# wx-ys/pynbody-extras

Measured on AMD Instinct MI355X. Metric: particle-pairs/sec (direct-sum gravity, force+potential), higher is better.
Workload: dtype f64; 1 GPU; 1000000-particle Plummer sphere, direct-sum force+potential (Newtonian), 1000000 targets/GPU x 1000000 sources; n_particles=1000000, seed=1002, parallelism=targets sharded x1, device=gfx950 device (gfx950:sramecc+:xnack-, 256 CUs)

## Files before the change

pynbody-extras_amd/csrc/direct.hip:

```cpp
#include <cstdlib>
#include <cstring>

#include "pbx_common.h"

namespace pbx {

static constexpr double kR2Tiny = 2.2250738585072014e-308;
static constexpr int kBlock = 256;

__device__ __forceinline__ double rsqrt_nr(double x) {
  double y = __builtin_amdgcn_rsq(x);
  double e = __builtin_fma(-x * y, y, 1.0);
  return __builtin_fma(0.5 * y, e, y);
}

__device__ __forceinline__ double w2_inner(double u) {
  double u2 = u * u;
  if (u < 0.5) {
    double u4 = u2 * u2;
    double u5 = u4 * u;
    return (16.0 / 3.0) * u2 - (48.0 / 5.0) * u4 + (32.0 / 5.0) * u5 - 14.0 / 5.0;
  }
  double inv_u = 1.0 / u;
  double u3 = u2 * u;
  double u4 = u2 * u2;
  double u5 = u4 * u;
  return (1.0 / 15.0) * inv_u + (32.0 / 3.0) * u2 - 16.0 * u3 + (48.0 / 5.0) * u4 -
         (32.0 / 15.0) * u5 - 16.0 / 5.0;
}

__device__ __forceinline__ double w2p_inner(double u) {
  double u2 = u * u;
  double u3 = u2 * u;
  double u4 = u2 * u2;
  if (u < 0.5) return (32.0 / 3.0) * u - (192.0 / 5.0) * u3 + 32.0 * u4;
  return -(1.0 / 15.0) * (1.0 / u2) + (64.0 / 3.0) * u - 48.0 * u2 + (192.0 / 5.0) * u3 -
         (32.0 / 3.0) * u4;
}

template <int KERN, int WANT>
__device__ __forceinline__ void pair(double dx, double dy, double dz, double m, double h,
                                     double &ph, double &ax, double &ay, double &az) {
  double s2 = __builtin_fma(dx, dx, __builtin_fma(dy, dy, __builtin_fma(dz, dz, kR2Tiny)));
  const double s = (KERN == 0) ? __builtin_fma(h, h, s2) : s2;
  const double y0 = __builtin_amdgcn_rsq(s);
  const double w = y0 * __builtin_fma(-s, y0 * y0, 3.0);
  double mw = m * w;
  double g8 = mw * (w * w);
  if (KERN == 1) {
    double r = s2 * (0.5 * w);
    if (!(h <= 0.0) && !(r >= h)) {
      double hinv = 1.0 / h;
      double u = r * hinv;
      mw = -2.0 * m * (w2_inner(u) * hinv);
      g8 = 8.0 * m * (w2p_inner(u) * (hinv * hinv) / r);
    }
  }
  if (WANT & PBX_WANT_POT) ph += mw;
  if (WANT & PBX_WANT_ACC) {
    ax = __builtin_fma(g8, dx, ax);
    ay = __builtin_fma(g8, dy, ay);
    az = __builtin_fma(g8, dz, az);
  }
}

template <int KERN, int WANT, bool CHECK, int T>
__device__ __forceinline__ void sweep(const double4 *__restrict__ src,
                                      const double *__restrict__ src_h, bool has_h,
                                      int64_t j0, int64_t j1, const double (&xi)[T],
                                      const double (&yi)[T], const double (&zi)[T],
                                      const double (&hi)[T], const int64_t (&me)[T],
                                      double (&ph)[T], double (&ax)[T], double (&ay)[T],
                                      double (&az)[T]) {
#pragma unroll 4
  for (int64_t j = j0; j < j1; ++j) {
    const double4 s = src[j];
    double hj = 0.0;
    if (KERN >= 0) hj = has_h ? src_h[j] : 0.0;
#pragma unroll
    for (int k = 0; k < T; ++k) {
      double dx = s.x - xi[k];
      double dy = s.y - yi[k];
      double dz = s.z - zi[k];
      double m = s.w;
      double h = 0.0;
      if (KERN >= 0) h = __builtin_fmax(hi[k], hj);
      if (CHECK) {
        bool self = (j == me[k]);
        m = self ? 0.0 : m;
        dx = self ? 1.0 : dx;
        if (KERN >= 0) h = self ? 0.0 : h;
      }
      pair<KERN, WANT>(dx, dy, dz, m, h, ph[k], ax[k], ay[k], az[k]);
    }
  }
}

template <int KERN, int WANT, bool SELF, int T>
__global__ void __launch_bounds__(kBlock)
    direct_kernel(const double4 *__restrict__ src, const double *__restrict__ src_h,
                  int has_h, int64_t n_src, int64_t chunk, const double *__restrict__ tgt,
                  const double *__restrict__ tgt_h, int64_t n_tgt, int64_t self_offset,
                  double *__restrict__ pot_out, double *__restrict__ acc_out,
                  int64_t out_split_stride) {
  const int64_t tbase = (int64_t)blockIdx.x * (kBlock * T);
  const int64_t js = (int64_t)blockIdx.y * chunk;
  const int64_t je = (js + chunk < n_src) ? js + chunk : n_src;

  double xi[T], yi[T], zi[T], hi[T], ph[T], ax[T], ay[T], az[T];
  int64_t me[T];
#pragma unroll
  for (int k = 0; k < T; ++k) {
    int64_t t = tbase + k * kBlock + threadIdx.x;
    int64_t tc = t < n_tgt ? t : n_tgt - 1;
    xi[k] = tgt[3 * tc + 0];
    yi[k] = tgt[3 * tc + 1];
    zi[k] = tgt[3 * tc + 2];
    hi[k] = (SELF && KERN >= 0 && has_h) ? tgt_h[tc] : 0.0;
    me[k] = SELF ? self_offset + t : -1;
    ph[k] = ax[k] = ay[k] = az[k] = 0.0;
  }

  const bool hh = has_h != 0;
  if (SELF) {
    int64_t d0 = self_offset + tbase;
    int64_t d1 = d0 + kBlock * T;
    d0 = d0 < js ? js : (d0 > je ? je : d0);
    d1 = d1 < js ? js : (d1 > je ? je : d1);
    sweep<KERN, WANT, false, T>(src, src_h, hh, js, d0, xi, yi, zi, hi, me, ph, ax, ay, az);
    sweep<KERN, WANT, true, T>(src, src_h, hh, d0, d1, xi, yi, zi, hi, me, ph, ax, ay, az);
    sweep<KERN, WANT, false, T>(src, src_h, hh, d1, je, xi, yi, zi, hi, me, ph, ax, ay, az);
  } else {
    sweep<KERN, WANT, false, T>(src, src_h, hh, js, je, xi, yi, zi, hi, me, ph, ax, ay, az);
  }

  const int64_t soff = (int64_t)blockIdx.y * out_split_stride;
#pragma unroll
  for (int k = 0; k < T; ++k) {
    int64_t t = tbase + k * kBlock + threadIdx.x;
    if (t < n_tgt) {
      if (WANT & PBX_WANT_POT) pot_out[soff + t] = -0.5 * ph[k];
      if (WANT & PBX_WANT_ACC) {
        double *a = acc_out + 3 * (soff + t);
        a[0] = 0.125 * ax[k];
        a[1] = 0.125 * ay[k];
        a[2] = 0.125 * az[k];
      }
    }
  }
}

template <int WANT>
__global__ void __launch_bounds__(kBlock)
    reduce_splits(const double *__restrict__ pot_part, const double *__restrict__ acc_part,
                  int nsplit, int64_t n_tgt, double *__restrict__ pot,
                  double *__restrict__ acc) {
  int64_t t = (int64_t)blockIdx.x * kBlock + threadIdx.x;
  if (t >= n_tgt) return;
  if (WANT & PBX_WANT_POT) {
    double s = 0.0;
    for (int k = 0; k < nsplit; ++k) s += pot_part[(int64_t)k * n_tgt + t];
    pot[t] = s;
  }
  if (WANT & PBX_WANT_ACC) {
    double sx = 0.0, sy = 0.0, sz = 0.0;
    for (int k = 0; k < nsplit; ++k) {
      const double *a = acc_part + 3 * ((int64_t)k * n_tgt + t);
      sx += a[0];
      sy += a[1];
      sz += a[2];
    }
    acc[3 * t + 0] = sx;
    acc[3 * t + 1] = sy;
    acc[3 * t + 2] = sz;
  }
}

__global__ void __launch_bounds__(kBlock)
    pack_sources_kernel(const double *__restrict__ pos, const double *__restrict__ mass,
                        int64_t n, double4 *__restrict__ rec) {
  int64_t i = (int64_t)blockIdx.x * kBlock + threadIdx.x;
  if (i >= n) return;
  rec[i] = make_double4(pos[3 * i + 0], pos[3 * i + 1], pos[3 * i + 2],
                        mass ? mass[i] : 1.0);
}

constexpr int kTargetsPerLane = 4;

template <int KERN, int WANT, bool SELF>
static void launch_variant(hipStream_t st, dim3 grid, const double4 *src, const double *src_h,
                           int has_h, int64_t n_src, int64_t chunk, const double *tgt,
                           const double *tgt_h, int64_t n_tgt, int64_t self_offset,
                           double *pot, double *acc, int64_t stride) {
  hipLaunchKernelGGL((direct_kernel<KERN, WANT, SELF, kTargetsPerLane>), grid, dim3(kBlock), 0,
                     st, src, src_h, has_h, n_src, chunk, tgt, tgt_h, n_tgt, self_offset, pot, acc,
                     stride);
}

template <int KERN, int WANT>
static void launch_self(bool self, hipStream_t st, dim3 grid, const double4 *src,
                        const double *src_h, int has_h, int64_t n_src, int64_t chunk,
                        const double *tgt, const double *tgt_h, int64_t n_tgt,
                        int64_t self_offset, double *pot, double *acc, int64_t stride) {
  if (self)
    launch_variant<KERN, WANT, true>(st, grid, src, src_h, has_h, n_src, chunk, tgt, tgt_h,
                                     n_tgt, self_offset, pot, acc, stride);
  else
    launch_variant<KERN, WANT, false>(st, grid, src, src_h, has_h, n_src, chunk, tgt, tgt_h,
                                      n_tgt, self_offset, pot, acc, stride);
}

template <int KERN>
static void launch_want(int want, bool self, hipStream_t st, dim3 grid, const double4 *src,
                        const double *src_h, int has_h, int64_t n_src, int64_t chunk,
                        const double *tgt, const double *tgt_h, int64_t n_tgt,
                        int64_t self_offset, double *pot, double *acc, int64_t stride) {
  switch (want) {
    case 1:
      launch_self<KERN, 1>(self, st, grid, src, src_h, has_h, n_src, chunk, tgt, tgt_h, n_tgt,
                           self_offset, pot, acc, stride);
      break;
    case 2:
      launch_self<KERN, 2>(self, st, grid, src, src_h, has_h, n_src, chunk, tgt, tgt_h, n_tgt,
                           self_offset, pot, acc, stride);
      break;
    default:
      launch_self<KERN, 3>(self, st, grid, src, src_h, has_h, n_src, chunk, tgt, tgt_h, n_tgt,
                           self_offset, pot, acc, stride);
      break;
  }
}

int64_t sym_padded(int64_t n);
int64_t sym_unit_count(int64_t n);
void sym_accumulate(Device &d, double4 *rec, int64_t n, int64_t u0, int64_t u1, int want,
                    double *acc4, DevBuf &unit_buf);
void sym_finish(Device &d, const double *acc4, int64_t lo, int64_t hi, int want, double *pot,
                double *acc);

static constexpr int64_t kSymMinN = 8192;

void direct_device(Device &d, const double *src, const double *src_h, int64_t n_src,
                   const double *tgt, const double *tgt_h, int64_t n_tgt, int64_t self_offset,
                   int kernel, int want, double *pot, double *acc) {
  if (n_tgt <= 0) return;
  hipStream_t st = d.stream;
  if (kernel == PBX_KERNEL_NONE && self_offset == 0 && n_tgt == n_src && n_src >= kSymMinN) {
    const int64_t npad = sym_padded(n_src);
    double4 *rec = (double4 *)d.slot(kSlotSymRec).ensure(sizeof(double4) * npad);
    double *acc4 = (double *)d.slot(kSlotSymAcc).ensure(sizeof(double) * 4 * npad);
    PBX_HIP(hipMemcpyAsync(rec, src, sizeof(double4) * n_src, hipMemcpyDeviceToDevice, st));
    PBX_HIP(hipMemsetAsync(acc4, 0, sizeof(double) * 4 * npad, st));
    sym_accumulate(d, rec, n_src, 0, sym_unit_count(n_src), want, acc4, d.slot(kSlotSymUnits));
    sym_finish(d, acc4, 0, n_src, want, pot, acc);
    return;
  }
  if (n_src <= 0) {
    if (want & PBX_WANT_POT) PBX_HIP(hipMemsetAsync(pot, 0, sizeof(double) * n_tgt, st));
    if (want & PBX_WANT_ACC) PBX_HIP(hipMemsetAsync(acc, 0, sizeof(double) * 3 * n_tgt, st));
    return;
  }
  const int64_t per_block = (int64_t)kBlock * kTargetsPerLane;
  const int64_t bx = (n_tgt + per_block - 1) / per_block;
  int64_t nsplit = (2048 + bx - 1) / bx;
  int64_t max_split = (n_src + 4095) / 4096;
  if (nsplit > max_split) nsplit = max_split;
  if (nsplit > 64) nsplit = 64;
  if (nsplit < 1) nsplit = 1;
  const int64_t chunk = (n_src + nsplit - 1) / nsplit;
  nsplit = (n_src + chunk - 1) / chunk;
  if (bx > 0x7fffffff) fail(PBX_ERR_VALUE, "too many targets (%lld)", (long long)n_tgt);
  dim3 grid((unsigned)bx, (unsigned)nsplit);
  const bool self = self_offset >= 0;
  const int has_h = src_h != nullptr;

  double *pot_k = pot, *acc_k = acc;
  int64_t stride = 0;
  if (nsplit > 1) {
    size_t per = 0;
    if (want & PBX_WANT_POT) per += 1;
    if (want & PBX_WANT_ACC) per += 3;
    double *part = (double *)d.slot(kSlotPart).ensure(sizeof(double) * per * nsplit * n_tgt);
    pot_k = (want & PBX_WANT_POT) ? part : nullptr;
    acc_k = (want & PBX_WANT_ACC) ? part + ((want & PBX_WANT_POT) ? nsplit * n_tgt : 0)
                                  : nullptr;
    stride = n_tgt;
  }
  const double4 *src4 = (const double4 *)src;
  switch (kernel) {
    case PBX_KERNEL_NONE:
      launch_want<-1>(want, self, st, grid, src4, src_h, has_h, n_src, chunk, tgt, tgt_h,
                      n_tgt, self_offset, pot_k, acc_k, stride);
      break;
    case PBX_KERNEL_PLUMMER:
      launch_want<0>(want, self, st, grid, src4, src_h, has_h, n_src, chunk, tgt, tgt_h,
                     n_tgt, self_offset, pot_k, acc_k, stride);
      break;
    case PBX_KERNEL_SPLINE:
      launch_want<1>(want, self, st, grid, src4, src_h, has_h, n_src, chunk, tgt, tgt_h,
                     n_tgt, self_offset, pot_k, acc_k, stride);
      break;
    default:
      fail(PBX_ERR_VALUE, "kernel must be 0 (Plummer) or 1 (CubicSplineW2)");
  }
  PBX_HIP(hipGetLastError());
  if (nsplit > 1) {
    dim3 rg(ceil_div(n_tgt, kBlock));
    switch (want) {
      case 1:
        hipLaunchKernelGGL(reduce_splits<1>, rg, dim3(kBlock), 0, st, pot_k, acc_k,
                           (int)nsplit, n_tgt, pot, acc);
        break;
      case 2:
        hipLaunchKernelGGL(reduce_splits<2>, rg, dim3(kBlock), 0, st, pot_k, acc_k,
                           (int)nsplit, n_tgt, pot, acc);
        break;
      default:
        hipLaunchKernelGGL(reduce_splits<3>, rg, dim3(kBlock), 0, st, pot_k, acc_k,
                           (int)nsplit, n_tgt, pot, acc);
        break;
    }
    PBX_HIP(hipGetLastError());
  }
}

void pack_sources_device(Device &d, const double *pos, const double *mass, int64_t n,
                         double *rec) {
  if (n <= 0) return;
  hipLaunchKernelGGL(pack_sources_kernel, dim3(ceil_div(n, kBlock)), dim3(kBlock), 0, d.stream,
                     pos, mass, n, (double4 *)rec);
  PBX_HIP(hipGetLastError());
}

static void check_kernel(int kernel, const double *soft) {
  if (kernel != PBX_KERNEL_NONE && kernel != PBX_KERNEL_PLUMMER && kernel != PBX_KERNEL_SPLINE)
    fail(PBX_ERR_VALUE, "kernel must be 0 (Plummer) or 1 (CubicSplineW2)");
  if (kernel == PBX_KERNEL_NONE && soft != nullptr)
    fail(PBX_ERR_VALUE,
         "softenings require an explicit kernel; pass kernel=0/1 (or omit softenings)");
}

static void direct_host(const double *h_pos, int64_t n, const double *h_tgt, int64_t m,
                        const double *h_mass, const double *h_soft, int kernel, int want,
                        double *h_out) {
  if (n < 0 || m < 0) fail(PBX_ERR_VALUE, "negative particle count");
  check_kernel(kernel, h_soft);
  const bool self = (h_tgt == nullptr);
  const int64_t n_tgt = self ? n : m;
  if (n_tgt == 0) return;
  Device &d = current_device();
  std::lock_guard<std::mutex> lk(d.mu);
  hipStream_t st = d.stream;
  size_t out_elems = (want == PBX_WANT_POT ? 1 : 3) * (size_t)n_tgt;
  if (n == 0) {
    std::memset(h_out, 0, sizeof(double) * out_elems);
    return;
  }
  ScopedTimer total("pbx.direct.total");
  double *d_pos = (double *)d.slot(kSlotPos).ensure(sizeof(double) * 3 * n);
  double *d_mass = h_mass ? (double *)d.slot(kSlotMass).ensure(sizeof(double) * n) : nullptr;
  double *d_src = (double *)d.slot(kSlotSrc).ensure(sizeof(double) * 4 * n);
  const bool use_h = h_soft != nullptr && kernel != PBX_KERNEL_NONE;
  double *d_src_h = use_h ? (double *)d.slot(kSlotSrcH).ensure(sizeof(double) * n) : nullptr;
  double *d_tgt = self ? d_pos : (double *)d.slot(kSlotTgt).ensure(sizeof(double) * 3 * m);
  double *d_out = (double *)d.slot(want == PBX_WANT_POT ? kSlotPot : kSlotAcc)
                      .ensure(sizeof(double) * out_elems);
  {
    ScopedTimer t("pbx.direct.h2d");
    PBX_HIP(hipMemcpyAsync(d_pos, h_pos, sizeof(double) * 3 * n, hipMemcpyHostToDevice, st));
    if (h_mass)
      PBX_HIP(hipMemcpyAsync(d_mass, h_mass, sizeof(double) * n, hipMemcpyHostToDevice, st));
    if (use_h)
      PBX_HIP(hipMemcpyAsync(d_src_h, h_soft, sizeof(double) * n, hipMemcpyHostToDevice, st));
    if (!self)
      PBX_HIP(hipMemcpyAsync(d_tgt, h_tgt, sizeof(double) * 3 * m, hipMemcpyHostToDevice, st));
    if (timing_enabled()) PBX_HIP(hipStreamSynchronize(st));
  }
  {
    ScopedTimer t("pbx.direct.compute");
    pack_sources_device(d, d_pos, d_mass, n, d_src);
    direct_device(d, d_src, d_src_h, n, d_tgt, self ? d_src_h : nullptr, n_tgt,
                  self ? 0 : -1, kernel, want, want == PBX_WANT_POT ? d_out : nullptr,
                  want == PBX_WANT_ACC ? d_out : nullptr);
    if (timing_enabled()) PBX_HIP(hipStreamSynchronize(st));
  }
  {
    ScopedTimer t("pbx.direct.d2h");
    PBX_HIP(hipMemcpyAsync(h_out, d_out, sizeof(double) * out_elems, hipMemcpyDeviceToHost, st));
    PBX_HIP(hipStreamSynchronize(st));
  }
}

}

using namespace pbx;

extern "C" {

int pbx_direct_accelerations(const double *h_pos, int64_t n, const double *h_masses,
                             const double *h_softenings, int kernel, double *h_acc) {
  return guard([&] {
    direct_host(h_pos, n, nullptr, 0, h_masses, h_softenings, kernel, PBX_WANT_ACC, h_acc);
  });
}

int pbx_direct_potentials(const double *h_pos, int64_t n, const double *h_masses,
                          const double *h_softenings, int kernel, double *h_pot) {
  return guard([&] {
    direct_host(h_pos, n, nullptr, 0, h_masses, h_softenings, kernel, PBX_WANT_POT, h_pot);
  });
}

int pbx_direct_accelerations_at_points(const double *h_pos, int64_t n, const double *h_targets,
                                       int64_t m, const double *h_masses,
                                       const double *h_softenings, int kernel, double *h_acc) {
  return guard([&] {
    if (m > 0 && !h_targets) fail(PBX_ERR_VALUE, "targets must be (N,3) float64 array");
    direct_host(h_pos, n, h_targets ? h_targets : h_pos, m, h_masses, h_softenings, kernel,
                PBX_WANT_ACC, h_acc);
  });
}

int pbx_direct_potentials_at_points(const double *h_pos, int64_t n, const double *h_targets,
                                    int64_t m, const double *h_masses,
                                    const double *h_softenings, int kernel, double *h_pot) {
  return guard([&] {
    if (m > 0 && !h_targets) fail(PBX_ERR_VALUE, "targets must be (N,3) float64 array");
    direct_host(h_pos, n, h_targets ? h_targets : h_pos, m, h_masses, h_softenings, kernel,
                PBX_WANT_POT, h_pot);
  });
}

int pbx_pack_sources(const double *d_pos, const double *d_mass, int64_t n, double *d_records) {
  return guard([&] {
    if (n < 0) fail(PBX_ERR_VALUE, "negative particle count");
    Device &d = current_device();
    pack_sources_device(d, d_pos, d_mass, n, d_records);
  });
}

int pbx_direct_dev(const double *d_src, const double *d_src_h, int64_t n_src,
                   const double *d_tgt, const double *d_tgt_h, int64_t n_tgt,
                   int64_t self_offset, int kernel, int want, double *d_pot, double *d_acc) {
  return guard([&] {
    if (n_src < 0 || n_tgt < 0) fail(PBX_ERR_VALUE, "negative particle count");
    if (want < 1 || want > 3) fail(PBX_ERR_VALUE, "want must be 1 (pot), 2 (acc) or 3");
    if ((want & PBX_WANT_POT) && !d_pot && n_tgt) fail(PBX_ERR_VALUE, "d_pot is NULL");
    if ((want & PBX_WANT_ACC) && !d_acc && n_tgt) fail(PBX_ERR_VALUE, "d_acc is NULL");
    if (kernel != PBX_KERNEL_NONE && kernel != PBX_KERNEL_PLUMMER && kernel != PBX_KERNEL_SPLINE)
      fail(PBX_ERR_VALUE, "kernel must be 0 (Plummer) or 1 (CubicSplineW2)");
    if (self_offset >= 0 && self_offset + n_tgt > n_src)
      fail(PBX_ERR_VALUE, "self_offset + n_tgt exceeds n_src");
    if (self_offset >= 0 && kernel != PBX_KERNEL_NONE && d_src_h && !d_tgt_h)
      fail(PBX_ERR_VALUE, "all-particles softened form needs d_tgt_h");
    Device &d = current_device();
    std::lock_guard<std::mutex> lk(d.mu);
    direct_device(d, d_src, kernel == PBX_KERNEL_NONE ? nullptr : d_src_h, n_src, d_tgt,
                  d_tgt_h, n_tgt, self_offset, kernel, want, d_pot, d_acc);
  });
}

}
```

pynbody-extras_amd/csrc/direct_sym.hip:

```cpp
#include <algorithm>
#include <type_traits>
#include <vector>

#include "pbx_common.h"

namespace pbx {
namespace sym {

static constexpr double kR2Tiny = 2.2250738585072014e-308;
constexpr int kWaves = 4;
#ifndef PBX_SYM_KT
#define PBX_SYM_KT 12
#endif
#ifndef PBX_SYM_KS
#define PBX_SYM_KS 2
#endif
constexpr int kT = PBX_SYM_KT;
constexpr int kS = PBX_SYM_KS;
constexpr int kBlk = 64 * kT;
constexpr int kChunk = 64 * kS;
constexpr int kJPerI = kBlk / kChunk;
constexpr int kSuper = kWaves * kBlk;
static_assert(kJPerI * kChunk == kBlk, "an I-block is a whole number of J-chunks");

struct Unit {
  int32_t sb;
  int32_t j0;
  int32_t j1;
  int32_t pad;
};

__device__ __forceinline__ double rot(double v, int addr) {
  const uint64_t b = __builtin_bit_cast(uint64_t, v);
  const int lo = __builtin_amdgcn_ds_bpermute(addr, (int)(uint32_t)b);
  const int hi = __builtin_amdgcn_ds_bpermute(addr, (int)(uint32_t)(b >> 32));
  return __builtin_bit_cast(double, ((uint64_t)(uint32_t)hi << 32) | (uint64_t)(uint32_t)lo);
}

__device__ __forceinline__ double rot_dpp(double v) {
  const uint64_t b = __builtin_bit_cast(uint64_t, v);
  const int l0 = (int)(uint32_t)b, h0 = (int)(uint32_t)(b >> 32);
  const int lo = __builtin_amdgcn_update_dpp(l0, l0, 0x134, 0xF, 0xF, false);
  const int hi = __builtin_amdgcn_update_dpp(h0, h0, 0x134, 0xF, 0xF, false);
  return __builtin_bit_cast(double, ((uint64_t)(uint32_t)hi << 32) | (uint64_t)(uint32_t)lo);
}
#ifndef PBX_SYM_DPP_MASK
#define PBX_SYM_DPP_MASK 0xFF
#endif

template <int WANT, bool SYMM, bool RAW, bool UNI, int DOFF = 0>
__device__ __forceinline__ void chunk(const double4 *__restrict__ rec, int64_t jbase, int lane,
                                      const double (&tx)[kT], const double (&ty)[kT],
                                      const double (&tz)[kT], const double (&tm)[kT],
                                      double (&tp)[kT], double (&ta)[kT], double (&tb)[kT],
                                      double (&tc)[kT], double (&sp)[kS], double (&sa)[kS],
                                      double (&sb)[kS], double (&sc)[kS]) {
  double sx[kS], sy[kS], sz[kS], sm[kS];
#pragma unroll
  for (int k = 0; k < kS; ++k) {
    const double4 r = rec[jbase + k * 64 + lane];
    sx[k] = r.x;
    sy[k] = r.y;
    sz[k] = r.z;
    sm[k] = UNI ? 0.0 : r.w;
    sp[k] = sa[k] = sb[k] = sc[k] = 0.0;
  }
  const int addr = ((lane + 1) & 63) << 2;
  for (int r = 0; r < 64; ++r) {
#pragma unroll
    for (int ks = 0; ks < kS; ++ks) {
#pragma unroll
      for (int kt = 0; kt < kT; ++kt) {
        double dx = sx[ks] - tx[kt], dy = sy[ks] - ty[kt], dz = sz[ks] - tz[kt];
        double ms = sm[ks];
        bool self = false;
        if (!SYMM && kt == DOFF * kS + ks) {
          self = (r == 0);
          ms = self ? 0.0 : ms;
          dx = self ? 1.0 : dx;
        }
        const double s2 =
            __builtin_fma(dx, dx, __builtin_fma(dy, dy, __builtin_fma(dz, dz, kR2Tiny)));
        const double y0 = __builtin_amdgcn_rsq(s2);
        double w = RAW ? y0 : y0 * __builtin_fma(-s2, y0 * y0, 3.0);
        if (UNI && !SYMM && kt == DOFF * kS + ks) w = self ? 0.0 : w;
        const double q = w * (w * w);
        if (WANT & PBX_WANT_POT) tp[kt] = UNI ? tp[kt] + w : __builtin_fma(ms, w, tp[kt]);
        if (WANT & PBX_WANT_ACC) {
          const double g = UNI ? q : ms * q;
          ta[kt] = __builtin_fma(g, dx, ta[kt]);
          tb[kt] = __builtin_fma(g, dy, tb[kt]);
          tc[kt] = __builtin_fma(g, dz, tc[kt]);
        }
        if (SYMM) {
          if (WANT & PBX_WANT_POT) sp[ks] = UNI ? sp[ks] + w : __builtin_fma(tm[kt], w, sp[ks]);
          if (WANT & PBX_WANT_ACC) {
            const double g = UNI ? q : tm[kt] * q;
            sa[ks] = __builtin_fma(-g, dx, sa[ks]);
            sb[ks] = __builtin_fma(-g, dy, sb[ks]);
            sc[ks] = __builtin_fma(-g, dz, sc[ks]);
          }
        }
      }
      auto rt = [&](double x, int bit) {
        return ((PBX_SYM_DPP_MASK >> bit) & 1) ? rot_dpp(x) : rot(x, addr);
      };
      sx[ks] = rt(sx[ks], 0);
      sy[ks] = rt(sy[ks], 1);
      sz[ks] = rt(sz[ks], 2);
      if (!UNI) sm[ks] = rt(sm[ks], 3);
      if (SYMM) {
        if (WANT & PBX_WANT_POT) sp[ks] = rt(sp[ks], 4);
        if (WANT & PBX_WANT_ACC) {
          sa[ks] = rt(sa[ks], 5);
          sb[ks] = rt(sb[ks], 6);
          sc[ks] = rt(sc[ks], 7);
        }
      }
    }
  }
}

template <int WANT, bool RAW, bool UNI, int D>
__device__ __forceinline__ void own_chunk(int d, const double4 *__restrict__ rec, int64_t jbase,
                                          int lane, const double (&tx)[kT], const double (&ty)[kT],
                                          const double (&tz)[kT], const double (&tm)[kT],
                                          double (&tp)[kT], double (&ta)[kT], double (&tb)[kT],
                                          double (&tc)[kT], double (&sp)[kS], double (&sa)[kS],
                                          double (&sb)[kS], double (&sc)[kS]) {
  if (d == D)
    chunk<WANT, false, RAW, UNI, D>(rec, jbase, lane, tx, ty, tz, tm, tp, ta, tb, tc, sp, sa, sb, sc);
  else if constexpr (D + 1 < kJPerI)
    own_chunk<WANT, RAW, UNI, D + 1>(d, rec, jbase, lane, tx, ty, tz, tm, tp, ta, tb, tc, sp, sa, sb,
                                     sc);
}

template <int WANT, bool RAW, bool UNI>
__global__ void __launch_bounds__(kWaves * 64)
    sym_kernel(const double4 *__restrict__ rec, const Unit *__restrict__ units,
               double *__restrict__ acc4, double m) {
  __shared__ double jl[kWaves][4][kChunk];
  const Unit u = units[blockIdx.x];
  const int w = threadIdx.x >> 6, lane = threadIdx.x & 63;
  const int64_t iblk = (int64_t)u.sb * kWaves + w;
  double tx[kT], ty[kT], tz[kT], tm[kT], tp[kT], ta[kT], tb[kT], tc[kT];
#pragma unroll
  for (int k = 0; k < kT; ++k) {
    const double4 r = rec[iblk * kBlk + k * 64 + lane];
    tx[k] = r.x;
    ty[k] = r.y;
    tz[k] = r.z;
    tm[k] = UNI ? 0.0 : r.w;
    tp[k] = ta[k] = tb[k] = tc[k] = 0.0;
  }
  const int64_t jdiag = iblk * kJPerI;
  for (int32_t j = u.j0; j < u.j1; ++j) {
    double sp[kS], sa[kS], sb[kS], sc[kS];
#pragma unroll
    for (int k = 0; k < kS; ++k) sp[k] = sa[k] = sb[k] = sc[k] = 0.0;
    if (j >= jdiag + kJPerI)
      chunk<WANT, true, RAW, UNI>(rec, (int64_t)j * kChunk, lane, tx, ty, tz, tm, tp, ta, tb, tc, sp,
                                  sa, sb, sc);
    else if (j >= jdiag)
      own_chunk<WANT, RAW, UNI, 0>((int)(j - jdiag), rec, (int64_t)j * kChunk, lane, tx, ty, tz, tm,
                                   tp, ta, tb, tc, sp, sa, sb, sc);
#pragma unroll
    for (int k = 0; k < kS; ++k) {
      jl[w][0][k * 64 + lane] = sp[k];
      jl[w][1][k * 64 + lane] = sa[k];
      jl[w][2][k * 64 + lane] = sb[k];
      jl[w][3][k * 64 + lane] = sc[k];
    }
    __syncthreads();
    if ((int64_t)j >= ((int64_t)u.sb * kWaves + 1) * kJPerI) {
      double *dst = acc4 + (int64_t)j * kChunk * 4;
      static_assert(kWaves * 64 * kS == kChunk * 4, "kS (source, quantity) words per thread");
#pragma unroll
      for (int i = 0; i < kS; ++i) {
        const int idx = threadIdx.x + i * kWaves * 64;
        const int s = idx >> 2, q = idx & 3;
        double v = jl[0][q][s] + jl[1][q][s] + jl[2][q][s] + jl[3][q][s];
        if (UNI) v *= m;
        if (v != 0.0) atomicAdd(dst + idx, v);
      }
    }
    __syncthreads();
  }
#pragma unroll
  for (int k = 0; k < kT; ++k) {
    double *dst = acc4 + (iblk * kBlk + k * 64 + lane) * 4;
    if (WANT & PBX_WANT_POT) atomicAdd(dst + 0, UNI ? m * tp[k] : tp[k]);
    if (WANT & PBX_WANT_ACC) {
      atomicAdd(dst + 1, UNI ? m * ta[k] : ta[k]);
      atomicAdd(dst + 2, UNI ? m * tb[k] : tb[k]);
      atomicAdd(dst + 3, UNI ? m * tc[k] : tc[k]);
    }
  }
}

__global__ void pad_records(double4 *__restrict__ rec, int64_t n, int64_t npad) {
  int64_t i = n + (int64_t)blockIdx.x * 256 + threadIdx.x;
  if (i >= npad) return;
  const double far = 1e100 * (double)(i - n + 1);
  rec[i] = make_double4(far, -far, 2.0 * far, 0.0);
}

struct MassProbe {
  double m;
  uint32_t differs;
  uint32_t pad;
};
__global__ void mass_probe(const double4 *__restrict__ rec, int64_t n,
                           MassProbe *__restrict__ out) {
  const int64_t i = (int64_t)blockIdx.x * 256 + threadIdx.x;
  const double m0 = rec[0].w;
  if (i == 0) out->m = m0;
  if (i < n && __builtin_bit_cast(uint64_t, rec[i].w) != __builtin_bit_cast(uint64_t, m0))
    out->differs = 1u;
}

__global__ void finish_kernel(const double *__restrict__ acc4, int64_t lo, int64_t hi, int want,
                              int raw, double *__restrict__ pot, double *__restrict__ acc) {
  int64_t t = (int64_t)blockIdx.x * 256 + threadIdx.x;
  if (lo + t >= hi) return;
  const double *a = acc4 + (lo + t) * 4;
  const double kp = raw ? -1.0 : -0.5, ka = raw ? 1.0 : 0.125;
  if (want & PBX_WANT_POT) pot[t] = kp * a[0];
  if (want & PBX_WANT_ACC) {
    acc[3 * t + 0] = ka * a[1];
    acc[3 * t + 1] = ka * a[2];
    acc[3 * t + 2] = ka * a[3];
  }
}

}

int64_t sym_padded(int64_t n) {
  return (n + sym::kSuper - 1) / sym::kSuper * sym::kSuper;
}

#ifndef PBX_SYM_CHUNKS_PER_UNIT
#define PBX_SYM_CHUNKS_PER_UNIT 32
#endif
static std::vector<sym::Unit> sym_units(int64_t npad) {
  constexpr int kChunksPerUnit = PBX_SYM_CHUNKS_PER_UNIT;
  const int32_t nch = (int32_t)(npad / sym::kChunk);
  const int32_t nsb = (int32_t)(npad / sym::kSuper);
  std::vector<sym::Unit> u;
  for (int32_t sb = 0; sb < nsb; ++sb)
    for (int32_t j = sb * sym::kWaves * sym::kJPerI; j < nch; j += kChunksPerUnit)
      u.push_back({sb, j, std::min(nch, j + kChunksPerUnit), 0});
  return u;
}

int64_t sym_unit_count(int64_t n) { return (int64_t)sym_units(sym_padded(n)).size(); }

static sym::MassProbe sym_probe_mass(Device &d, const double4 *rec, int64_t n) {
  hipStream_t st = d.stream;
  sym::MassProbe *dp = (sym::MassProbe *)d.slot(kSlotSymProbe).ensure(sizeof(sym::MassProbe));
  sym::MassProbe h{};
  const bool timed = timing_enabled();
  hipEvent_t e0 = nullptr, e1 = nullptr;
  if (timed) {
    PBX_HIP(hipEventCreate(&e0));
    PBX_HIP(hipEventCreate(&e1));
    PBX_HIP(hipEventRecord(e0, st));
  }
  PBX_HIP(hipMemsetAsync(dp, 0, sizeof(sym::MassProbe), st));
  hipLaunchKernelGGL(sym::mass_probe, dim3(ceil_div(n, 256)), dim3(256), 0, st, rec, n, dp);
  PBX_HIP(hipGetLastError());
  PBX_HIP(hipMemcpyAsync(&h, dp, sizeof(sym::MassProbe), hipMemcpyDeviceToHost, st));
  if (timed) PBX_HIP(hipEventRecord(e1, st));
  PBX_HIP(hipStreamSynchronize(st));
  if (timed) {
    float ms = 0.f;
    PBX_HIP(hipEventElapsedTime(&ms, e0, e1));
    std::fprintf(stderr, "[pynbodyext-timing] direct_sym mass probe (n=%lld): %.4f ms\n",
                 (long long)n, (double)ms);
    (void)hipEventDestroy(e0);
    (void)hipEventDestroy(e1);
  }
  return h;
}


void sym_accumulate(Device &d, double4 *rec, int64_t n, int64_t u0, int64_t u1, int want,
                    double *acc4, DevBuf &unit_buf) {
  const int64_t npad = sym_padded(n);
  hipStream_t st = d.stream;
  if (npad > n)
    hipLaunchKernelGGL(sym::pad_records, dim3(ceil_div(npad - n, 256)), dim3(256), 0, st, rec, n,
                       npad);
  std::vector<sym::Unit> all = sym_units(npad);
  u0 = std::max<int64_t>(0, u0);
  u1 = std::min<int64_t>((int64_t)all.size(), u1);
  if (u1 <= u0) return;
  std::vector<sym::Unit> mine(all.begin() + u0, all.begin() + u1);
  std::stable_sort(mine.begin(), mine.end(), [](const sym::Unit &a, const sym::Unit &b) {
    return (a.j1 - a.j0) > (b.j1 - b.j0);
  });
  sym::Unit *du = (sym::Unit *)unit_buf.ensure(sizeof(sym::Unit) * mine.size());
  PBX_HIP(hipMemcpyAsync(du, mine.data(), sizeof(sym::Unit) * mine.size(), hipMemcpyHostToDevice,
                         st));
  const sym::MassProbe probe = sym_probe_mass(d, rec, n);
  const bool uni = probe.differs == 0;
  const double m = probe.m;
  const dim3 grid((unsigned)mine.size()), block(sym::kWaves * 64);
  auto launch = [&](auto raw, auto uniform) {
    constexpr bool R = decltype(raw)::value, U = decltype(uniform)::value;
    if (want == PBX_WANT_POT)
      hipLaunchKernelGGL((sym::sym_kernel<PBX_WANT_POT, R, U>), grid, block, 0, st, rec, du, acc4,
                         m);
    else if (want == PBX_WANT_ACC)
      hipLaunchKernelGGL((sym::sym_kernel<PBX_WANT_ACC, R, U>), grid, block, 0, st, rec, du, acc4,
                         m);
    else
      hipLaunchKernelGGL((sym::sym_kernel<PBX_WANT_POT | PBX_WANT_ACC, R, U>), grid, block, 0, st,
                         rec, du, acc4, m);
  };
  auto launch_raw = [&](auto raw) {
    if (uni)
      launch(raw, std::true_type{});
    else
      launch(raw, std::false_type{});
  };
  if (precise_mode())
    launch_raw(std::false_type{});
  else
    launch_raw(std::true_type{});
  ++(uni ? d.sym_uniform_launches : d.sym_general_launches);
  PBX_HIP(hipGetLastError());
  PBX_HIP(hipStreamSynchronize(st));
}

void sym_finish(Device &d, const double *acc4, int64_t lo, int64_t hi, int want, double *pot,
                double *acc) {
  if (hi <= lo) return;
  hipLaunchKernelGGL(sym::finish_kernel, dim3(ceil_div(hi - lo, 256)), dim3(256), 0, d.stream,
                     acc4, lo, hi, want, precise_mode() ? 0 : 1, pot, acc);
  PBX_HIP(hipGetLastError());
}

}

using namespace pbx;

extern "C" {

int pbx_direct_sym_plan(int64_t n, int64_t *npad, int64_t *n_units, int64_t *h_weights) {
  return guard([&] {
    if (n < 0) fail(PBX_ERR_VALUE, "negative particle count");
    const int64_t np = sym_padded(n);
    std::vector<sym::Unit> u = sym_units(np);
    if (npad) *npad = np;
    if (n_units) *n_units = (int64_t)u.size();
    if (h_weights)
      for (size_t i = 0; i < u.size(); ++i) h_weights[i] = u[i].j1 - u[i].j0;
  });
}

int pbx_direct_sym_accumulate(const double *d_src, int64_t n, int64_t u0, int64_t u1, int want,
                              double *d_acc4) {
  return guard([&] {
    if (n < 0) fail(PBX_ERR_VALUE, "negative particle count");
    if (want < 1 || want > 3) fail(PBX_ERR_VALUE, "want must be 1 (pot), 2 (acc) or 3");
    if (n == 0) return;
    Device &d = current_device();
    std::lock_guard<std::mutex> lk(d.mu);
    const int64_t npad = sym_padded(n);
    double4 *rec = (double4 *)d.slot(kSlotSymRec).ensure(sizeof(double4) * npad);
    PBX_HIP(hipMemcpyAsync(rec, d_src, sizeof(double4) * n, hipMemcpyDeviceToDevice, d.stream));
    sym_accumulate(d, rec, n, u0, u1, want, d_acc4, d.slot(kSlotSymUnits));
  });
}

int pbx_direct_sym_path_stats(int64_t *uniform_launches, int64_t *general_launches) {
  return guard([&] {
    Device &d = current_device();
    std::lock_guard<std::mutex> lk(d.mu);
    if (uniform_launches) *uniform_launches = d.sym_uniform_launches;
    if (general_launches) *general_launches = d.sym_general_launches;
  });
}

int pbx_direct_sym_finish(const double *d_acc4, int64_t lo, int64_t hi, int want, double *d_pot,
                          double *d_acc) {
  return guard([&] {
    if (lo < 0 || hi < lo) fail(PBX_ERR_VALUE, "bad particle range");
    Device &d = current_device();
    std::lock_guard<std::mutex> lk(d.mu);
    sym_finish(d, d_acc4, lo, hi, want, d_pot, d_acc);
    PBX_HIP(hipStreamSynchronize(d.stream));
  });
}

}
```

pynbody-extras_amd/csrc/pbx_common.h:

```cpp
#pragma once

#include <hip/hip_runtime.h>

#include <chrono>
#include <condition_variable>
#include <cstdarg>
#include <cstdint>
#include <cstdio>
#include <mutex>
#include <string>
#include <thread>
#include <vector>

#include "../../include/pbx.h"

namespace pbx {

void set_error(const char *fmt, ...);

struct Error {
  int code;
  std::string msg;
};

[[noreturn]] void fail(int code, const char *fmt, ...);

#define PBX_HIP(call)                                                        \
  do {                                                                       \
    hipError_t _e = (call);                                                  \
    if (_e != hipSuccess)                                                    \
      ::pbx::fail(PBX_ERR_RUNTIME, "%s failed: %s (%s:%d)", #call,           \
                  hipGetErrorString(_e), __FILE__, __LINE__);                \
  } while (0)

template <class F> int guard(F &&f) {
  try {
    f();
    return PBX_OK;
  } catch (const Error &e) {
    set_error("%s", e.msg.c_str());
    return e.code;
  } catch (const std::bad_alloc &) {
    set_error("host allocation failed");
    return PBX_ERR_RUNTIME;
  } catch (...) {
    set_error("unknown internal error");
    return PBX_ERR_RUNTIME;
  }
}

struct DevBuf {
  void *ptr = nullptr;
  size_t bytes = 0;
  void *ensure(size_t need);
  ~DevBuf();
};

void *dev_alloc(size_t need, size_t *got, int *dev);
void dev_release(void *p, size_t bytes, int dev);

struct Device {
  int id = -1;
  hipStream_t stream = nullptr;
  std::mutex mu;
  std::vector<DevBuf *> slots;
  DevBuf &slot(int k);
  std::vector<void *> ring;
  std::vector<hipEvent_t> ring_ev;
  std::vector<bool> ring_used;
  int64_t sym_uniform_launches = 0, sym_general_launches = 0;
};

enum Slot {
  kSlotSrc = 0,
  kSlotSrcH,
  kSlotTgt,
  kSlotTgtH,
  kSlotPos,
  kSlotMass,
  kSlotPot,
  kSlotAcc,
  kSlotPart,
  kSlotProf0,
  kSlotProf1,
  kSlotProf2,
  kSlotProf3,
  kSlotProf4,
  kSlotProf5,
  kSlotProf6,
  kSlotProf7,
  kSlotComm,
  kSlotSymRec,
  kSlotSymAcc,
  kSlotSymUnits,
  kSlotSymProbe,
  kSlotPropPos,
  kSlotPropVel,
  kSlotPropMass,
  kSlotPropPart,
  kSlotCount
};

Device &current_device();

void h2d_staged(Device &d, void *dst, const void *src, size_t bytes, hipStream_t st);
void d2h_staged(Device &d, void *dst, const void *src, size_t bytes, hipStream_t st);
bool d2h_staged_widen(Device &d, int64_t *dst, const int32_t *src, int64_t n, hipStream_t st);

bool timing_enabled();

struct ScopedTimer {
  const char *label;
  std::chrono::steady_clock::time_point t0;
  bool on;
  explicit ScopedTimer(const char *l)
      : label(l), t0(std::chrono::steady_clock::now()), on(timing_enabled()) {}
  ~ScopedTimer() {
    if (on) {
      double ms = std::chrono::duration<double, std::milli>(
                      std::chrono::steady_clock::now() - t0)
                      .count();
      std::fprintf(stderr, "[pynbodyext-timing] %s: %.3f ms\n", label, ms);
    }
  }
};

struct CommRanks {
  int nranks, rank;
};
CommRanks comm_ranks(void *comm);
void comm_allreduce(void *comm, const void *send, void *recv, int64_t count, int dtype, int op,
                    hipStream_t st, std::unique_lock<std::mutex> &lk);

bool precise_mode();
void set_precise_mode(bool on);

inline unsigned int ceil_div(int64_t a, int64_t b) {
  return (unsigned int)((a + b - 1) / b);
}

constexpr unsigned kNumXcd = 8;
__device__ __forceinline__ unsigned xcd_swizzle(unsigned b, unsigned nblocks) {
  const unsigned q = nblocks / kNumXcd, r = nblocks % kNumXcd;
  const unsigned x = b % kNumXcd, k = b / kNumXcd;
  return (x < r ? x * (q + 1) : r * (q + 1) + (x - r) * q) + k;
}
__device__ __forceinline__ unsigned xcd_chunk_swizzle(unsigned b, unsigned chunk) {
  const unsigned x = b % kNumXcd, k = b / kNumXcd;
  return ((k / chunk) * kNumXcd + x) * chunk + k % chunk;
}

}
```

Before: 3563 billion pairs/s.

## Add separate uniform-mass tile shape, cache unit tables, drop trailing sync

Templatizes the symmetric pair kernel on a tile shape so the uniform-mass path can use its own KT/KS, clipping rows past n when its superblock differs. Unit tables are cached per device in pinned host memory and reused across calls instead of being rebuilt and copied every time. The final stream synchronize in sym_accumulate is removed. By default the uniform tile equals the general one, so the main gains come from lower host overhead; a missing sync could expose ordering issues for callers that relied on it.

```diff
diff --git a/pynbody-extras_amd/csrc/direct.hip b/pynbody-extras_amd/csrc/direct.hip
--- a/pynbody-extras_amd/csrc/direct.hip
+++ b/pynbody-extras_amd/csrc/direct.hip
@@ -232,9 +232,10 @@
 }
 
 int64_t sym_padded(int64_t n);
+int64_t sym_rec_padded(int64_t n);
 int64_t sym_unit_count(int64_t n);
 void sym_accumulate(Device &d, double4 *rec, int64_t n, int64_t u0, int64_t u1, int want,
-                    double *acc4, DevBuf &unit_buf);
+                    double *acc4);
 void sym_finish(Device &d, const double *acc4, int64_t lo, int64_t hi, int want, double *pot,
                 double *acc);
 
@@ -247,11 +248,12 @@
   hipStream_t st = d.stream;
   if (kernel == PBX_KERNEL_NONE && self_offset == 0 && n_tgt == n_src && n_src >= kSymMinN) {
     const int64_t npad = sym_padded(n_src);
-    double4 *rec = (double4 *)d.slot(kSlotSymRec).ensure(sizeof(double4) * npad);
+    double4 *rec =
+        (double4 *)d.slot(kSlotSymRec).ensure(sizeof(double4) * sym_rec_padded(n_src));
     double *acc4 = (double *)d.slot(kSlotSymAcc).ensure(sizeof(double) * 4 * npad);
     PBX_HIP(hipMemcpyAsync(rec, src, sizeof(double4) * n_src, hipMemcpyDeviceToDevice, st));
     PBX_HIP(hipMemsetAsync(acc4, 0, sizeof(double) * 4 * npad, st));
-    sym_accumulate(d, rec, n_src, 0, sym_unit_count(n_src), want, acc4, d.slot(kSlotSymUnits));
+    sym_accumulate(d, rec, n_src, 0, sym_unit_count(n_src), want, acc4);
     sym_finish(d, acc4, 0, n_src, want, pot, acc);
     return;
   }
diff --git a/pynbody-extras_amd/csrc/direct_sym.hip b/pynbody-extras_amd/csrc/direct_sym.hip
--- a/pynbody-extras_amd/csrc/direct_sym.hip
+++ b/pynbody-extras_amd/csrc/direct_sym.hip
@@ -15,13 +15,24 @@
 #ifndef PBX_SYM_KS
 #define PBX_SYM_KS 2
 #endif
-constexpr int kT = PBX_SYM_KT;
-constexpr int kS = PBX_SYM_KS;
-constexpr int kBlk = 64 * kT;
-constexpr int kChunk = 64 * kS;
-constexpr int kJPerI = kBlk / kChunk;
-constexpr int kSuper = kWaves * kBlk;
-static_assert(kJPerI * kChunk == kBlk, "an I-block is a whole number of J-chunks");
+#ifndef PBX_SYM_UNI_KT
+#define PBX_SYM_UNI_KT PBX_SYM_KT
+#endif
+#ifndef PBX_SYM_UNI_KS
+#define PBX_SYM_UNI_KS PBX_SYM_KS
+#endif
+template <int KT, int KS>
+struct Tile {
+  static constexpr int kT = KT;
+  static constexpr int kS = KS;
+  static constexpr int kBlk = 64 * KT;
+  static constexpr int kChunk = 64 * KS;
+  static constexpr int kJPerI = kBlk / kChunk;
+  static constexpr int kSuper = kWaves * kBlk;
+  static_assert(kJPerI * kChunk == kBlk, "an I-block is a whole number of J-chunks");
+};
+using GenTile = Tile<PBX_SYM_KT, PBX_SYM_KS>;
+using UniTile = Tile<PBX_SYM_UNI_KT, PBX_SYM_UNI_KS>;
 
 struct Unit {
   int32_t sb;
@@ -48,13 +59,14 @@
 #define PBX_SYM_DPP_MASK 0xFF
 #endif
 
-template <int WANT, bool SYMM, bool RAW, bool UNI, int DOFF = 0>
+template <class T, int WANT, bool SYMM, bool RAW, bool UNI, int DOFF = 0>
 __device__ __forceinline__ void chunk(const double4 *__restrict__ rec, int64_t jbase, int lane,
-                                      const double (&tx)[kT], const double (&ty)[kT],
-                                      const double (&tz)[kT], const double (&tm)[kT],
-                                      double (&tp)[kT], double (&ta)[kT], double (&tb)[kT],
-                                      double (&tc)[kT], double (&sp)[kS], double (&sa)[kS],
-                                      double (&sb)[kS], double (&sc)[kS]) {
+                                      const double (&tx)[T::kT], const double (&ty)[T::kT],
+                                      const double (&tz)[T::kT], const double (&tm)[T::kT],
+                                      double (&tp)[T::kT], double (&ta)[T::kT], double (&tb)[T::kT],
+                                      double (&tc)[T::kT], double (&sp)[T::kS], double (&sa)[T::kS],
+                                      double (&sb)[T::kS], double (&sc)[T::kS]) {
+  constexpr int kT = T::kT, kS = T::kS;
   double sx[kS], sy[kS], sz[kS], sm[kS];
 #pragma unroll
   for (int k = 0; k < kS; ++k) {
@@ -121,24 +133,25 @@
   }
 }
 
-template <int WANT, bool RAW, bool UNI, int D>
+template <class T, int WANT, bool RAW, bool UNI, int D>
 __device__ __forceinline__ void own_chunk(int d, const double4 *__restrict__ rec, int64_t jbase,
-                                          int lane, const double (&tx)[kT], const double (&ty)[kT],
-                                          const double (&tz)[kT], const double (&tm)[kT],
-                                          double (&tp)[kT], double (&ta)[kT], double (&tb)[kT],
-                                          double (&tc)[kT], double (&sp)[kS], double (&sa)[kS],
-                                          double (&sb)[kS], double (&sc)[kS]) {
+                                          int lane, const double (&tx)[T::kT], const double (&ty)[T::kT],
+                                          const double (&tz)[T::kT], const double (&tm)[T::kT],
+                                          double (&tp)[T::kT], double (&ta)[T::kT], double (&tb)[T::kT],
+                                          double (&tc)[T::kT], double (&sp)[T::kS], double (&sa)[T::kS],
+                                          double (&sb)[T::kS], double (&sc)[T::kS]) {
   if (d == D)
-    chunk<WANT, false, RAW, UNI, D>(rec, jbase, lane, tx, ty, tz, tm, tp, ta, tb, tc, sp, sa, sb, sc);
-  else if constexpr (D + 1 < kJPerI)
-    own_chunk<WANT, RAW, UNI, D + 1>(d, rec, jbase, lane, tx, ty, tz, tm, tp, ta, tb, tc, sp, sa, sb,
-                                     sc);
-}
-
-template <int WANT, bool RAW, bool UNI>
+    chunk<T, WANT, false, RAW, UNI, D>(rec, jbase, lane, tx, ty, tz, tm, tp, ta, tb, tc, sp, sa, sb, sc);
+  else if constexpr (D + 1 < T::kJPerI)
+    own_chunk<T, WANT, RAW, UNI, D + 1>(d, rec, jbase, lane, tx, ty, tz, tm, tp, ta, tb, tc, sp, sa,
+                                        sb, sc);
+}
+
+template <class T, int WANT, bool RAW, bool UNI, bool CLIP>
 __global__ void __launch_bounds__(kWaves * 64)
     sym_kernel(const double4 *__restrict__ rec, const Unit *__restrict__ units,
-               double *__restrict__ acc4, double m) {
+               double *__restrict__ acc4, double m, int64_t nrow) {
+  constexpr int kT = T::kT, kS = T::kS, kBlk = T::kBlk, kChunk = T::kChunk, kJPerI = T::kJPerI;
   __shared__ double jl[kWaves][4][kChunk];
   const Unit u = units[blockIdx.x];
   const int w = threadIdx.x >> 6, lane = threadIdx.x & 63;
@@ -159,11 +172,11 @@
 #pragma unroll
     for (int k = 0; k < kS; ++k) sp[k] = sa[k] = sb[k] = sc[k] = 0.0;
     if (j >= jdiag + kJPerI)
-      chunk<WANT, true, RAW, UNI>(rec, (int64_t)j * kChunk, lane, tx, ty, tz, tm, tp, ta, tb, tc, sp,
-                                  sa, sb, sc);
+      chunk<T, WANT, true, RAW, UNI>(rec, (int64_t)j * kChunk, lane, tx, ty, tz, tm, tp, ta, tb, tc,
+                                     sp, sa, sb, sc);
     else if (j >= jdiag)
-      own_chunk<WANT, RAW, UNI, 0>((int)(j - jdiag), rec, (int64_t)j * kChunk, lane, tx, ty, tz, tm,
-                                   tp, ta, tb, tc, sp, sa, sb, sc);
+      own_chunk<T, WANT, RAW, UNI, 0>((int)(j - jdiag), rec, (int64_t)j * kChunk, lane, tx, ty, tz,
+                                      tm, tp, ta, tb, tc, sp, sa, sb, sc);
 #pragma unroll
     for (int k = 0; k < kS; ++k) {
       jl[w][0][k * 64 + lane] = sp[k];
@@ -181,6 +194,7 @@
         const int s = idx >> 2, q = idx & 3;
         double v = jl[0][q][s] + jl[1][q][s] + jl[2][q][s] + jl[3][q][s];
         if (UNI) v *= m;
+        if (CLIP && (int64_t)j * kChunk + s >= nrow) v = 0.0;
         if (v != 0.0) atomicAdd(dst + idx, v);
       }
     }
@@ -188,7 +202,9 @@
   }
 #pragma unroll
   for (int k = 0; k < kT; ++k) {
-    double *dst = acc4 + (iblk * kBlk + k * 64 + lane) * 4;
+    const int64_t row = iblk * kBlk + k * 64 + lane;
+    if (CLIP && row >= nrow) continue;
+    double *dst = acc4 + row * 4;
     if (WANT & PBX_WANT_POT) atomicAdd(dst + 0, UNI ? m * tp[k] : tp[k]);
     if (WANT & PBX_WANT_ACC) {
       atomicAdd(dst + 1, UNI ? m * ta[k] : ta[k]);
@@ -235,25 +251,77 @@
 
 }
 
-int64_t sym_padded(int64_t n) {
-  return (n + sym::kSuper - 1) / sym::kSuper * sym::kSuper;
+template <class T>
+static int64_t padded(int64_t n) {
+  return (n + T::kSuper - 1) / T::kSuper * T::kSuper;
+}
+
+int64_t sym_padded(int64_t n) { return padded<sym::GenTile>(n); }
+
+int64_t sym_rec_padded(int64_t n) {
+  return std::max(padded<sym::GenTile>(n), padded<sym::UniTile>(n));
 }
 
 #ifndef PBX_SYM_CHUNKS_PER_UNIT
 #define PBX_SYM_CHUNKS_PER_UNIT 32
 #endif
+template <class T>
+static constexpr int chunks_per_unit() {
+  constexpr int c = PBX_SYM_CHUNKS_PER_UNIT * sym::GenTile::kChunk / T::kChunk;
+  return c > 0 ? c : 1;
+}
+template <class T>
 static std::vector<sym::Unit> sym_units(int64_t npad) {
-  constexpr int kChunksPerUnit = PBX_SYM_CHUNKS_PER_UNIT;
-  const int32_t nch = (int32_t)(npad / sym::kChunk);
-  const int32_t nsb = (int32_t)(npad / sym::kSuper);
+  constexpr int kChunksPerUnit = chunks_per_unit<T>();
+  const int32_t nch = (int32_t)(npad / T::kChunk);
+  const int32_t nsb = (int32_t)(npad / T::kSuper);
   std::vector<sym::Unit> u;
   for (int32_t sb = 0; sb < nsb; ++sb)
-    for (int32_t j = sb * sym::kWaves * sym::kJPerI; j < nch; j += kChunksPerUnit)
+    for (int32_t j = sb * sym::kWaves * T::kJPerI; j < nch; j += kChunksPerUnit)
       u.push_back({sb, j, std::min(nch, j + kChunksPerUnit), 0});
   return u;
 }
-
-int64_t sym_unit_count(int64_t n) { return (int64_t)sym_units(sym_padded(n)).size(); }
+template <class T>
+static int64_t unit_count(int64_t npad) {
+  constexpr int kChunksPerUnit = chunks_per_unit<T>();
+  const int64_t nch = npad / T::kChunk, nsb = npad / T::kSuper;
+  int64_t c = 0;
+  for (int64_t sb = 0; sb < nsb; ++sb)
+    c += (nch - sb * sym::kWaves * T::kJPerI + kChunksPerUnit - 1) / kChunksPerUnit;
+  return c;
+}
+
+int64_t sym_unit_count(int64_t n) { return unit_count<sym::GenTile>(sym_padded(n)); }
+
+template <class T>
+static const sym::Unit *unit_table(Device &d, int which, int64_t npad, int64_t u0, int64_t u1) {
+  SymUnitTable &t = d.sym_tables[which];
+  if (t.dev && t.npad == npad && t.u0 == u0 && t.u1 == u1) return (const sym::Unit *)t.dev;
+  std::vector<sym::Unit> all = sym_units<T>(npad);
+  std::vector<sym::Unit> mine(all.begin() + u0, all.begin() + u1);
+  std::stable_sort(mine.begin(), mine.end(), [](const sym::Unit &a, const sym::Unit &b) {
+    return (a.j1 - a.j0) > (b.j1 - b.j0);
+  });
+  const size_t bytes = sizeof(sym::Unit) * mine.size();
+  t.dev = nullptr;
+  if (t.host) PBX_HIP(hipStreamSynchronize(d.stream));
+  if (bytes > t.host_bytes) {
+    if (t.host) (void)hipHostFree(t.host);
+    t.host = nullptr;
+    t.host_bytes = 0;
+    const size_t want = (bytes + 65535) & ~(size_t)65535;
+    PBX_HIP(hipHostMalloc(&t.host, want, hipHostMallocDefault));
+    t.host_bytes = want;
+  }
+  std::copy(mine.begin(), mine.end(), (sym::Unit *)t.host);
+  void *dev = d.slot(which ? kSlotSymUnitsUni : kSlotSymUnits).ensure(bytes);
+  PBX_HIP(hipMemcpyAsync(dev, t.host, bytes, hipMemcpyHostToDevice, d.stream));
+  t.npad = npad;
+  t.u0 = u0;
+  t.u1 = u1;
+  t.dev = dev;
+  return (const sym::Unit *)dev;
+}
 
 static sym::MassProbe sym_probe_mass(Device &d, const double4 *rec, int64_t n) {
   hipStream_t st = d.stream;
@@ -284,53 +352,63 @@
 }
 
 
+template <class T, bool UNI, bool CLIP>
+static void launch_sym(hipStream_t st, int64_t units, int want, bool raw, const double4 *rec,
+                       const sym::Unit *du, double *acc4, double m, int64_t n) {
+  const dim3 grid((unsigned)units), block(sym::kWaves * 64);
+  auto launch = [&](auto r) {
+    constexpr bool R = decltype(r)::value;
+    if (want == PBX_WANT_POT)
+      hipLaunchKernelGGL((sym::sym_kernel<T, PBX_WANT_POT, R, UNI, CLIP>), grid, block, 0, st, rec,
+                         du, acc4, m, n);
+    else if (want == PBX_WANT_ACC)
+      hipLaunchKernelGGL((sym::sym_kernel<T, PBX_WANT_ACC, R, UNI, CLIP>), grid, block, 0, st, rec,
+                         du, acc4, m, n);
+    else
+      hipLaunchKernelGGL((sym::sym_kernel<T, PBX_WANT_POT | PBX_WANT_ACC, R, UNI, CLIP>), grid,
+                         block, 0, st, rec, du, acc4, m, n);
+  };
+  if (raw)
+    launch(std::true_type{});
+  else
+    launch(std::false_type{});
+}
+
 void sym_accumulate(Device &d, double4 *rec, int64_t n, int64_t u0, int64_t u1, int want,
-                    double *acc4, DevBuf &unit_buf) {
-  const int64_t npad = sym_padded(n);
+                    double *acc4) {
+  using sym::GenTile;
+  using sym::UniTile;
   hipStream_t st = d.stream;
-  if (npad > n)
-    hipLaunchKernelGGL(sym::pad_records, dim3(ceil_div(npad - n, 256)), dim3(256), 0, st, rec, n,
-                       npad);
-  std::vector<sym::Unit> all = sym_units(npad);
+  const int64_t npad = padded<GenTile>(n), all = unit_count<GenTile>(npad);
+  const bool whole = u0 <= 0 && u1 >= all;
   u0 = std::max<int64_t>(0, u0);
-  u1 = std::min<int64_t>((int64_t)all.size(), u1);
+  u1 = std::min<int64_t>(all, u1);
   if (u1 <= u0) return;
-  std::vector<sym::Unit> mine(all.begin() + u0, all.begin() + u1);
-  std::stable_sort(mine.begin(), mine.end(), [](const sym::Unit &a, const sym::Unit &b) {
-    return (a.j1 - a.j0) > (b.j1 - b.j0);
-  });
-  sym::Unit *du = (sym::Unit *)unit_buf.ensure(sizeof(sym::Unit) * mine.size());
-  PBX_HIP(hipMemcpyAsync(du, mine.data(), sizeof(sym::Unit) * mine.size(), hipMemcpyHostToDevice,
-                         st));
   const sym::MassProbe probe = sym_probe_mass(d, rec, n);
-  const bool uni = probe.differs == 0;
+  const bool uni = probe.differs == 0, raw = !precise_mode();
   const double m = probe.m;
-  const dim3 grid((unsigned)mine.size()), block(sym::kWaves * 64);
-  auto launch = [&](auto raw, auto uniform) {
-    constexpr bool R = decltype(raw)::value, U = decltype(uniform)::value;
-    if (want == PBX_WANT_POT)
-      hipLaunchKernelGGL((sym::sym_kernel<PBX_WANT_POT, R, U>), grid, block, 0, st, rec, du, acc4,
-                         m);
-    else if (want == PBX_WANT_ACC)
-      hipLaunchKernelGGL((sym::sym_kernel<PBX_WANT_ACC, R, U>), grid, block, 0, st, rec, du, acc4,
-                         m);
+  const bool wide = uni && whole;
+  const int64_t np = wide ? padded<UniTile>(n) : npad;
+  if (np > n)
+    hipLaunchKernelGGL(sym::pad_records, dim3(ceil_div(np - n, 256)), dim3(256), 0, st, rec, n, np);
+  if (wide) {
+    const int64_t units = unit_count<UniTile>(np);
+    const sym::Unit *du = unit_table<UniTile>(d, 1, np, 0, units);
+    constexpr bool kClip = UniTile::kSuper != GenTile::kSuper;
+    launch_sym<UniTile, true, kClip>(st, units, want, raw, rec, du, acc4, m, n);
+  } else {
+    const sym::Unit *du = unit_table<GenTile>(d, 0, np, u0, u1);
+    if (uni)
+      launch_sym<GenTile, true, false>(st, u1 - u0, want, raw, rec, du, acc4, m, n);
     else
-      hipLaunchKernelGGL((sym::sym_kernel<PBX_WANT_POT | PBX_WANT_ACC, R, U>), grid, block, 0, st,
-                         rec, du, acc4, m);
-  };
-  auto launch_raw = [&](auto raw) {
-    if (uni)
-      launch(raw, std::true_type{});
-    else
-      launch(raw, std::false_type{});
-  };
-  if (precise_mode())
-    launch_raw(std::false_type{});
-  else
-    launch_raw(std::true_type{});
+      launch_sym<GenTile, false, false>(st, u1 - u0, want, raw, rec, du, acc4, m, n);
+  }
   ++(uni ? d.sym_uniform_launches : d.sym_general_launches);
   PBX_HIP(hipGetLastError());
-  PBX_HIP(hipStreamSynchronize(st));
+  if (timing_enabled())
+    std::fprintf(stderr, "[pynbodyext-timing] direct_sym tile (n=%lld, %s masses): %d x %d\n",
+                 (long long)n, uni ? "uniform" : "general", wide ? UniTile::kT : GenTile::kT,
+                 wide ? UniTile::kS : GenTile::kS);
 }
 
 void sym_finish(Device &d, const double *acc4, int64_t lo, int64_t hi, int want, double *pot,
@@ -351,7 +429,7 @@
   return guard([&] {
     if (n < 0) fail(PBX_ERR_VALUE, "negative particle count");
     const int64_t np = sym_padded(n);
-    std::vector<sym::Unit> u = sym_units(np);
+    std::vector<sym::Unit> u = sym_units<sym::GenTile>(np);
     if (npad) *npad = np;
     if (n_units) *n_units = (int64_t)u.size();
     if (h_weights)
@@ -367,10 +445,9 @@
     if (n == 0) return;
     Device &d = current_device();
     std::lock_guard<std::mutex> lk(d.mu);
-    const int64_t npad = sym_padded(n);
-    double4 *rec = (double4 *)d.slot(kSlotSymRec).ensure(sizeof(double4) * npad);
+    double4 *rec = (double4 *)d.slot(kSlotSymRec).ensure(sizeof(double4) * sym_rec_padded(n));
     PBX_HIP(hipMemcpyAsync(rec, d_src, sizeof(double4) * n, hipMemcpyDeviceToDevice, d.stream));
-    sym_accumulate(d, rec, n, u0, u1, want, d_acc4, d.slot(kSlotSymUnits));
+    sym_accumulate(d, rec, n, u0, u1, want, d_acc4);
   });
 }
 
diff --git a/pynbody-extras_amd/csrc/pbx_common.h b/pynbody-extras_amd/csrc/pbx_common.h
--- a/pynbody-extras_amd/csrc/pbx_common.h
+++ b/pynbody-extras_amd/csrc/pbx_common.h
@@ -59,6 +59,13 @@
 void *dev_alloc(size_t need, size_t *got, int *dev);
 void dev_release(void *p, size_t bytes, int dev);
 
+struct SymUnitTable {
+  int64_t npad = -1, u0 = 0, u1 = 0;
+  void *dev = nullptr;
+  void *host = nullptr;
+  size_t host_bytes = 0;
+};
+
 struct Device {
   int id = -1;
   hipStream_t stream = nullptr;
@@ -69,6 +76,7 @@
   std::vector<hipEvent_t> ring_ev;
   std::vector<bool> ring_used;
   int64_t sym_uniform_launches = 0, sym_general_launches = 0;
+  SymUnitTable sym_tables[2];
 };
 
 enum Slot {
@@ -93,6 +101,7 @@
   kSlotSymRec,
   kSlotSymAcc,
   kSlotSymUnits,
+  kSlotSymUnitsUni,
   kSlotSymProbe,
   kSlotPropPos,
   kSlotPropVel,
```

Measured after the change: 3570 billion pairs/s (median of 6 runs). About the same (+0.2%).
